# Nicolas-Zamorano/pytorch_fem_solver

Measured on AMD Instinct MI355X. Metric: Melements/s assembled (global K + f), higher is better.
Workload: dtype f64

## Files before the change

### include/tfem_assembly.h

```cpp
#ifndef TFEM_ASSEMBLY_H
#define TFEM_ASSEMBLY_H

#include <stdint.h>

#ifdef __cplusplus
extern "C" {
#endif

#define TFEM_ABI_VERSION 2

typedef enum tfem_status {
  TFEM_OK = 0,
  TFEM_ERR_INVALID_ARGUMENT = 1,
  TFEM_ERR_UNSUPPORTED = 2,
  TFEM_ERR_HIP = 3,
  TFEM_ERR_INDEX_RANGE = 4,
  TFEM_ERR_NO_DEVICE = 5
} tfem_status;

int tfem_abi_version(void);
const char *tfem_status_string(int status);
const char *tfem_last_error(void);
int tfem_device_count(void);
int tfem_quadrature_size(int quad_order);
// ... 125 lines not shown
  TFEM_SRC_SIN = 17, TFEM_SRC_COS = 18, TFEM_SRC_EXP = 19, TFEM_SRC_SQRT = 20,
  TFEM_SRC_LOG = 21, TFEM_SRC_TANH = 22,
  TFEM_SRC_OP_COUNT = 23
};
typedef struct tfem_source_program {
  int32_t n_ops;
  int32_t reserved;
  uint8_t ops[TFEM_SOURCE_MAX_OPS];
  double consts[TFEM_SOURCE_MAX_OPS];
} tfem_source_program;

int tfem_source_validate(const tfem_source_program *program);

int tfem_source_eval(const void *coords, int real_bytes, const void *conn, int idx_bytes,
                     int64_t n_elems, int64_t n_verts, int quad_order,
                     const tfem_source_program *program, void *fq, void *stream);

int tfem_p1_assemble_rings_source(const void *coords, int real_bytes, int64_t n_verts,
                                  int quad_order, double alpha, double beta,
                                  const void *plan_device, const int64_t *plan_layout_host,
                                  void *vals, int64_t nnz, const tfem_source_program *source,
                                  int64_t n_elems, void *fout, void *stream);

int tfem_p1_rings_coef(const void *coords, int real_bytes, int64_t n_verts, int quad_order,
                       double alpha, double beta, const tfem_source_program *kappa,
                       const tfem_source_program *c, const void *plan_device,
                       const int64_t *plan_layout_host, void *vals, void *stream);
int tfem_p1_apply_rings_coef(const void *coords, int real_bytes, int64_t n_verts, int quad_order,
                             double alpha, double beta, const tfem_source_program *kappa,
                             const tfem_source_program *c, const void *plan_device,
                             const int64_t *plan_layout_host, const void *u, void *y, void *stream);
int tfem_p1_apply_rings_coef_multi(const void *coords, int real_bytes, int64_t n_verts, int quad_order,
                                   double alpha, double beta, const tfem_source_program *kappa,
                                   const tfem_source_program *c, const void *plan_device,
                                   const int64_t *plan_layout_host, const void *u, void *y,
                                   int64_t n_vec, void *stream);

int tfem_p1_rings_field(const void *coords, int real_bytes, int64_t n_verts, int quad_order,
                        double alpha, double beta, const void *kappa, int kappa_nq, const void *c,
                        int c_nq, int64_t n_elems, const void *plan_device,
                        const int64_t *plan_layout_host, void *vals, void *stream);
int tfem_p1_apply_rings_field(const void *coords, int real_bytes, int64_t n_verts, int quad_order,
                              double alpha, double beta, const void *kappa, int kappa_nq,
                              const void *c, int c_nq, int64_t n_elems, const void *plan_device,
                              const int64_t *plan_layout_host, const void *u, void *y, void *stream);
int tfem_p1_field_adjoint(const void *coords, int real_bytes, const void *conn, int64_t n_elems,
// ... 70 lines not shown
```

### pytorch_fem_solver_amd/_native.py

```python

from __future__ import annotations

import ctypes
import os
from ctypes import c_char_p, c_double, c_int, c_int64, c_void_p

_HERE = os.path.dirname(os.path.abspath(__file__))
LIB_PATH = os.environ.get("TFEM_HIP_LIB") or os.path.join(_HERE, "csrc", "libtfem_hip.so")

_lib = None

ABI_VERSION = 2

SOURCE_MAX_OPS = 32
SOURCE_STACK = 4


class SourceProgram(ctypes.Structure):
    _fields_ = [
        ("n_ops", ctypes.c_int32),
        ("reserved", ctypes.c_int32),
        ("ops", ctypes.c_uint8 * SOURCE_MAX_OPS),
        ("consts", ctypes.c_double * SOURCE_MAX_OPS),
    ]
# ... 147 lines not shown
        c_int,
        [c_void_p, c_int, c_void_p, c_void_p, c_void_p, c_int64, c_int, c_void_p, c_void_p, c_void_p,
         c_void_p, c_void_p, c_int64, c_void_p],
    ),
    "tfem_edge_interpolate_p1_fracture": (
        c_int,
        [c_void_p, c_void_p, c_int, c_void_p, c_void_p, c_void_p, c_void_p, c_int64, c_int64, c_int64,
         c_int64, c_int, c_void_p, c_int64, c_void_p, c_void_p, c_void_p],
    ),
    "tfem_csr_gather_map": (c_int, [c_void_p, c_int64, c_int, c_int64, c_void_p, c_void_p]),
    "tfem_csr_gather": (c_int, [c_void_p, c_int, c_void_p, c_void_p, c_int64, c_void_p, c_void_p]),
    "tfem_interface_pack": (
        c_int,
        [c_void_p, c_void_p, c_int, c_void_p, c_void_p, c_int64, c_void_p, c_void_p, c_int64,
         c_void_p, c_int64, c_void_p],
    ),
    "tfem_interface_unpack": (
        c_int,
        [c_void_p, c_void_p, c_int, c_void_p, c_void_p, c_int64, c_void_p, c_void_p, c_int64,
         c_void_p, c_void_p],
    ),
    "tfem_interface_pack_dense": (c_int, [c_void_p, c_void_p, c_int, c_void_p, c_int64, c_void_p, c_void_p]),
    "tfem_source_validate": (c_int, [c_void_p]),
    "tfem_source_eval": (
        c_int,
        [c_void_p, c_int, c_void_p, c_int, c_int64, c_int64, c_int, c_void_p, c_void_p, c_void_p],
    ),
    "tfem_p1_assemble_rings_source": (
        c_int,
        [c_void_p, c_int, c_int64, c_int, c_double, c_double, c_void_p, c_void_p, c_void_p,
         c_int64, c_void_p, c_int64, c_void_p, c_void_p],
    ),
    "tfem_p1_rings_coef": (
        c_int,
        [c_void_p, c_int, c_int64, c_int, c_double, c_double, c_void_p, c_void_p, c_void_p, c_void_p,
         c_void_p, c_void_p],
    ),
    "tfem_p1_apply_rings_coef": (
        c_int,
        [c_void_p, c_int, c_int64, c_int, c_double, c_double, c_void_p, c_void_p, c_void_p, c_void_p,
         c_void_p, c_void_p, c_void_p],
    ),
    "tfem_p1_apply_rings_coef_multi": (
        c_int,
        [c_void_p, c_int, c_int64, c_int, c_double, c_double, c_void_p, c_void_p, c_void_p, c_void_p,
         c_void_p, c_void_p, c_int64, c_void_p],
# ... 79 lines not shown
```

### pytorch_fem_solver_amd/basis/engine.py

```python

from __future__ import annotations

import ctypes
import os
from ctypes import c_void_p

import numpy as np
import torch

from .. import _native
from ..sparse import CSRMatrix


class NoDeviceError(RuntimeError):
    pass


def _is_block(u):
    return u is not None and u.dim() == 2 and u.shape[1] > 1


def _compute_device(home: torch.device) -> torch.device:
    if home.type == "cuda":
        return home
    if torch.cuda.is_available():
        return torch.device("cuda", torch.cuda.current_device())
# ... 850 lines not shown
        out = torch.empty(out_len, dtype=self.dtype, device=self.device)
        with torch.cuda.device(self.device):
            _native.check(
                self.lib.tfem_tri_bilinear_csr(
                    _native.ptr(d["coords"]), self.real_bytes, _native.ptr(d["conn_geo"]), 4,
                    self.n_elems, self.coords_per_mesh, self.poly_order, self.quad_order,
                    float(alpha), float(beta), None if two_pass else _native.ptr(csr[2]),
                    _native.ptr(out), out_len,
                    _native.ptr(d["pinv"]), _native.ptr(d["fdet"]), self.n_fractures,
                    self.coords_per_mesh, self._stream(),
                )
            )
        return self._gather_local(out) if two_pass else out

    def _output(self, given, numel, what):
        if given is None:
            return torch.empty(numel, dtype=self.dtype, device=self.device)
        if (given.dtype != self.dtype or given.device != self.device or given.numel() != numel
                or not given.is_contiguous()):
            raise ValueError(f"out: {what} must be a contiguous {self.dtype} tensor of {numel} "
                             f"entries on {self.device}")
        return given.view(-1)

    def _assemble_rings(self, alpha, beta, fq=None, want_matrix=True, out=(None, None), source=None,
                        tiles=None):
        d = self._inputs()
        rings = self.ring_plan()
        nnz = int(self.csr_structure()[1].shape[0])
        vals = self._output(out[0], nnz, "CSR values") if want_matrix else None
        fout = None
        with_load = fq is not None or source is not None
        if fq is not None:
            fq = fq.to(self.device, self.dtype).reshape(self.n_elems, self.n_quad).contiguous()
        if with_load:
            fout = self._output(out[1], self.n_dofs, "load vector")
        with torch.cuda.device(self.device):
            if tiles is not None:
                _native.check(
                    self.lib.tfem_p1_assemble_rings_range(
                        _native.ptr(d["coords"]), self.real_bytes, self.n_dofs, self.quad_order,
                        float(alpha), float(beta), _native.ptr(rings["blob"]),
                        c_void_p(rings["layout"].ctypes.data), _native.ptr(vals), nnz,
                        _native.ptr(fq), ctypes.byref(source) if source is not None else None,
                        self.n_elems, _native.ptr(fout), int(tiles[0]), int(tiles[1]), self._stream(),
                    )
                )
            elif source is not None:
                _native.check(
                    self.lib.tfem_p1_assemble_rings_source(
                        _native.ptr(d["coords"]), self.real_bytes, self.n_dofs, self.quad_order,
                        float(alpha), float(beta), _native.ptr(rings["blob"]),
                        c_void_p(rings["layout"].ctypes.data), _native.ptr(vals), nnz,
                        ctypes.byref(source), self.n_elems, _native.ptr(fout), self._stream(),
                    )
                )
            else:
                _native.check(
                    self.lib.tfem_p1_assemble_rings(
# ... 362 lines not shown
        if (fq is None) == (source is None):
            raise ValueError("prepared_system: source values fq OR a source program")
        rings = self.ring_plan() if self._use_rings() else None
        if rings is None or (source is not None and not self._rings_take_source()) or (source is None and not rings["fq_ok"]):
            raise NotImplementedError("prepared launches need the ring plan of this basis")
        d = self._inputs()
        nnz = int(self.csr_structure()[1].shape[0])
        vals = self._output(out[0], nnz, "CSR values")
        fout = self._output(out[1], self.n_dofs, "load vector")
        first, count = self.tile_range(tiles) if tiles is not None else (0, -1)
        if fq is not None:
            fq = fq.to(self.device, self.dtype).reshape(self.n_elems, self.n_quad).contiguous()
        program = None
        if source is not None:
            program = _native.SourceProgram()
            ctypes.memmove(ctypes.byref(program), ctypes.byref(source), ctypes.sizeof(program))
        fixed = (_native.ptr(d["coords"]), self.real_bytes, self.n_dofs, self.quad_order, float(alpha), float(beta),
                 _native.ptr(rings["blob"]), c_void_p(rings["layout"].ctypes.data), _native.ptr(vals), nnz,
                 _native.ptr(fq), ctypes.byref(program) if program is not None else None, self.n_elems,
                 _native.ptr(fout), int(first), int(count))
        keep = (d, rings, vals, fout, fq, program)
        launch_fn, device, check = self.lib.tfem_p1_assemble_rings_range, self.device, _native.check
        current_stream = torch.cuda.current_stream

        def launch(stream=None):
            handle = (stream if stream is not None else current_stream(device)).cuda_stream
            status = launch_fn(*fixed, c_void_p(handle))
            if status:
                check(status)
            return keep[2], keep[3]

        return launch

    def supports_source(self):
        return self.n_fractures == 0 and self._host_coords.dim() == 2

    def _rings_take_source(self):
        if self.kernel == "tiles" or not self._use_rings():
            return False
        if os.environ.get("TFEM_DETERMINISTIC", "0") not in ("", "0"):
            return False
        rings = self.ring_plan()
        return bool(rings["elems_staged"] and rings["has_tverts"])

    def source_values(self, program):
        d = self._inputs()
        fq = torch.empty((self.n_elems, self.n_quad), dtype=self.dtype, device=self.device)
        with torch.cuda.device(self.device):
# ... 293 lines not shown
```

### pytorch_fem_solver_amd/csrc/tfem_rings.hip

```cpp
#include <cmath>

#include "tfem_rings_kernel.hpp"

namespace tfem {

template <typename T, bool MASS>
__global__ __launch_bounds__(kRingBlock) void k_p1_long_rows(const T *coords, const unsigned char *plan,
                                                             unsigned off_long, int n_long, T *vals, T stiff_w,
                                                             T mass_d, T mass_o) {
  RingLongSlot<T> s;
  ring_long_slot<T, MASS, false>(coords, plan, off_long, n_long, stiff_w, mass_o, nullptr, s);
  if (!s.slot) return;
  T *out = vals + s.rec[1];
  out[int((s.rec[19 + s.i / 8] >> (4 * (s.i % 8))) & 15u)] = s.entry;
  if (s.i == 0) out[s.dpos] = ring_diag<T, MASS>(s.sum, s.dsum, mass_d, mass_o);
}

struct RingLaunch {
  const void *coords;
  int quad_order;
  double alpha, beta;
  const unsigned char *plan;
  const int64_t *layout;
  int64_t n_verts, nnz;
// ... 22 lines not shown
static void *pick_ring_q(int nq) {
  switch (nq) {
    case 0: return reinterpret_cast<void *>(k_p1_rings<T, SLOTS, MASS, CHUNK, 0, false>);
    case 1: return reinterpret_cast<void *>(k_p1_rings<T, SLOTS, MASS, CHUNK, 1, false>);
    case 3: return reinterpret_cast<void *>(k_p1_rings<T, SLOTS, MASS, CHUNK, 3, false>);
    case 4: return reinterpret_cast<void *>(k_p1_rings<T, SLOTS, MASS, CHUNK, 4, false>);
    case 6: return reinterpret_cast<void *>(k_p1_rings<T, SLOTS, MASS, CHUNK, 6, false>);
    default: return nullptr;
  }
}

template <typename T, int SLOTS, bool CHUNK>
static void *pick_ring_mass(bool kmat, bool mass, int nq) {
  if (!kmat) return pick_ring_load_only<T, SLOTS, CHUNK>(nq);
  return mass ? pick_ring_q<T, SLOTS, true, CHUNK>(nq) : pick_ring_q<T, SLOTS, false, CHUNK>(nq);
}

template <typename T>
static void *pick_ring_kernel(int slots, bool mass, bool chunk, int nq, bool src, bool kmat, bool wide) {
  if (src) return pick_ring_src_kernel<T>(slots, mass, chunk, nq, kmat, wide);
  if (slots == 7)
    return chunk ? pick_ring_mass<T, 7, true>(kmat, mass, nq) : pick_ring_mass<T, 7, false>(kmat, mass, nq);
  return chunk ? pick_ring_mass<T, 15, true>(kmat, mass, nq) : pick_ring_mass<T, 15, false>(kmat, mass, nq);
}

template <typename T>
static int launch_rings(const RingLaunch &L) {
  TriTables tables;
  if (!build_tri_tables(L.quad_order, int(sizeof(T)), &tables))
    return fail(TFEM_ERR_UNSUPPORTED, "Integration order not implemented");
  const int64_t *z = L.layout;
  if (z[0] == 0) return TFEM_OK;
  const bool src = L.source != nullptr;
  const bool load = L.fq != nullptr || src;
  const bool kmat = L.vals != nullptr;
  if (src && L.fq) return fail(TFEM_ERR_INVALID_ARGUMENT, "source values AND a source program");
  if (!kmat && !load) return fail(TFEM_ERR_INVALID_ARGUMENT, "nothing to assemble");
  if (!L.coords || !L.plan || (load && !L.fout)) return fail(TFEM_ERR_INVALID_ARGUMENT, "NULL pointer");
  RingArgs<T> a;
  int st = ring_args_init<T>(tables, z, L.coords, L.plan, L.n_verts, L.alpha, L.beta, a);
  if (st != TFEM_OK) return st;
  const int64_t rb = int64_t(sizeof(T));
  const int64_t extents[3] = {kmat ? L.nnz * rb : 0, (load && !src) ? L.n_elems * tables.nq * rb : 0,
                              load ? L.n_verts * rb : 0};
  st = check_extents("ring kernel", extents, 3);
  if (st != TFEM_OK) return st;
// ... 30 lines not shown
    auto near = [tol](double x, double y) { return std::fabs(x - y) <= tol; };
    bool ok = tables.hw[1] == tables.hw[2] && tables.hw[1] == tables.hw[3];
    for (int i = 0; i < 3; ++i) {
      ok = ok && near(tables.lam[0][i], c0);
      for (int q = 1; q < 4; ++q) ok = ok && near(tables.lam[q][i], i == at[q] ? aa : b);
    }
    if (!ok) return fail(TFEM_ERR_UNSUPPORTED, "the 4-point rule is not the reference's order-3 rule");
    a.qsym[0] = T(c0);
    a.qsym[1] = T(b);
    a.qsym[2] = T(d);
    a.qsym[3] = T(c0) * T(tables.hw[0]);
    a.qsym[4] = T(b) * T(tables.hw[1]);
    a.qsym[5] = T(d) * T(tables.hw[1]);
  }
  if (src) {
    if (z[20] == 0 || z[21] == 0)
      return fail(TFEM_ERR_UNSUPPORTED, "the ring plan carries no element vertex table (source programs)");
    a.off_tverts = unsigned(z[20]);
    a.off_chain = unsigned(z[24]);
    a.off_hin = unsigned(z[26]);
    a.chain_len = int(z[25]);
    if (a.chain_len < 1 || z[24] == 0 || z[26] == 0)
      return fail(TFEM_ERR_INVALID_ARGUMENT, "the ring plan carries no chain order (layout of an older build?)");
    st = src_convert<T>(L.source, &a.src);
    if (st != TFEM_OK) return st;
  }
  const int64_t t_first = L.tile_first, t_count = L.tile_count < 0 ? z[0] - L.tile_first : L.tile_count;
  if (t_first < 0 || t_count < 0 || t_first + t_count > z[0])
    return fail(TFEM_ERR_INVALID_ARGUMENT, "tile range [%lld, +%lld) outside the plan's %lld tiles",
                (long long)t_first, (long long)t_count, (long long)z[0]);
  if (kmat && z[23] > 0 && (t_first != 0 || t_count != z[0]))
    return fail(TFEM_ERR_UNSUPPORTED, "a ring plan with long rows is launched over all of its tiles: the rows of "
                "the vertices with 8 .. 15 neighbours are written by one launch over all of them");
  if (t_count == 0) return TFEM_OK;
  a.n_tiles = int(t_count);
  a.n_runs = 0;
  if (src) {
    a.u_first = int(t_first);
    if (z[28] > 0 && (t_first != 0 || t_count != z[0]))
      return fail(TFEM_ERR_UNSUPPORTED, "tile ranges need a plan built with flagged vertices (its blocks break between the ranges)");
    if (z[28] > 0) {
      a.n_runs = int(z[28]);
      a.off_runs = unsigned(z[30]);
    }
  } else {
    a.off_desc += 80u * unsigned(t_first);
  }
  const bool mass = L.beta != 0.0;
  const int slots = int(z[6]);
  a.lds_elem = load ? int(z[17]) : 0;
  const size_t lds = size_t(4 * a.lds_vert) * sizeof(T) +
                     (kmat ? size_t(kRingWaves) * size_t(64 * (slots + 1) + 2) * sizeof(T) : 0) +
                     (src ? size_t(3 * (a.lds_vert + 2)) * sizeof(T)
                          : load ? size_t(3 * a.lds_elem + 4) * sizeof(T) : 0);
  const bool chunk = z[13] != 0;
  a.plain_stores = !load;
  if (const char *v = std::getenv("TFEM_RINGS_STORES")) a.plain_stores = std::strcmp(v, "plain") == 0;
  bool wide = src && src_depth(L.source) <= 2;
  if (const char *v = std::getenv("TFEM_SRC_WIDE")) wide = wide && std::atoi(v) != 0;
  void *kernel = pick_ring_kernel<T>(slots, mass, chunk, load ? tables.nq : 0, src, kmat, wide);
  if (!kernel) return fail(TFEM_ERR_UNSUPPORTED, "Integration order not implemented");
  int per_cu = 0;
  st = resident_per_cu(kernel, kRingBlock, lds, &per_cu);
  if (st != TFEM_OK) return st;
  const int deal = a.xcd_interleave > 0 ? a.xcd_interleave : 1;
  int per = int((t_count + 8 * deal - 1) / (8 * deal)) * deal;
  if (src) {
    const int64_t first_block = t_first / a.chain_len, last_block = (t_first + t_count - 1) / a.chain_len;
    per = int((last_block - first_block + 1 + 7) / 8);
    if (a.n_runs > 0) per = (a.n_runs + 7) / 8;
  }
  if (L.blocks_per_cu > 0 && L.blocks_per_cu < per_cu) per_cu = L.blocks_per_cu;
  int cus = device_cu_count();
  if (const char *v = std::getenv("TFEM_RINGS_RESERVE_CUS")) cus = std::max(8, cus - 8 * std::max(0, std::atoi(v)));
  const int blocks = std::min(per * 8, (cus * per_cu / 8) * 8);
  const dim3 grid{unsigned(blocks)}, block{unsigned(kRingBlock)};
  void *params[] = {&a};
  hipError_t e = hipLaunchKernel(kernel, grid, block, params, lds, L.stream);
  if (e != hipSuccess) return fail(TFEM_ERR_HIP, "ring kernel launch: %s", hipGetErrorString(e));
  if (kmat && z[23] > 0) {
    const dim3 lgrid{unsigned((16 * z[23] + kRingBlock - 1) / kRingBlock)};
    if (mass)
// ... 11 lines not shown
static int ring_entry(const void *coords, int real_bytes, int64_t n_verts, int quad_order, double alpha,
                      double beta, const void *plan_device, const int64_t *plan_layout_host, void *vals,
                      int64_t nnz, const void *fq, const tfem_source_program *source, int64_t n_elems,
                      void *fout, int64_t tile_first, int64_t tile_count, void *stream) {
  if (real_bytes != 4 && real_bytes != 8)
    return fail(TFEM_ERR_INVALID_ARGUMENT, "real_bytes must be 4 or 8");
  if (!plan_layout_host) return fail(TFEM_ERR_INVALID_ARGUMENT, "plan_layout_host is NULL");
  RingLaunch L{coords, quad_order, alpha, beta, static_cast<const unsigned char *>(plan_device),
               plan_layout_host, n_verts, nnz, vals, static_cast<hipStream_t>(stream)};
  L.fq = fq;
  L.source = source;
  L.n_elems = n_elems;
  L.fout = fout;
  L.tile_first = tile_first;
  L.tile_count = tile_count;
  if (const char *v = std::getenv("TFEM_RINGS_PER_CU")) L.blocks_per_cu = std::atoi(v);
  return real_bytes == 8 ? launch_rings<double>(L) : launch_rings<float>(L);
}

}

extern "C" {

int tfem_ring_capacity(int what) {
  using namespace tfem;
  switch (what) {
    case 0: return kRingBlock;
    case 1: return kRingVertCap;
    default: return 0;
  }
}

int tfem_p1_assemble_rings(const void *coords, int real_bytes, int64_t n_verts, int quad_order,
                           double alpha, double beta, const void *plan_device,
                           const int64_t *plan_layout_host, void *vals, int64_t nnz,
                           const void *fq, int64_t n_elems, void *fout, void *stream) {
  return tfem::ring_entry(coords, real_bytes, n_verts, quad_order, alpha, beta, plan_device, plan_layout_host, vals,
                          nnz, fq, nullptr, n_elems, fout, 0, -1, stream);
}

int tfem_p1_assemble_rings_source(const void *coords, int real_bytes, int64_t n_verts, int quad_order,
                                  double alpha, double beta, const void *plan_device,
                                  const int64_t *plan_layout_host, void *vals, int64_t nnz,
                                  const tfem_source_program *source, int64_t n_elems, void *fout,
                                  void *stream) {
  if (!source) return tfem::fail(TFEM_ERR_INVALID_ARGUMENT, "NULL pointer");
// ... 15 lines not shown
```

### pytorch_fem_solver_amd/csrc/tfem_rings_host.cpp

```cpp
#include <algorithm>
#include <cmath>
#include <cstdlib>
#include <cstring>
#include <memory>
#include <numeric>
#include <vector>
#include <chrono>
#include <cstdio>

#include "tfem_common.hpp"
#include "tfem_threads.hpp"

namespace tfem {

constexpr int kRingDescStride = 20;
constexpr int kRingLayoutLen = 32;
constexpr int kRingElemCap = 768;
constexpr int kRingElemRuns = 8;
constexpr int kRingHaloCapHost = 256;

struct RingPlan {
  int slots = 7, words = 4;
  std::vector<int32_t> desc;
  std::vector<uint32_t> rows;
// ... 1016 lines not shown
      {layout[9], p->rows.data(), int64_t(p->rows.size()) * 4},
      {layout[10], p->rowstart.data(), int64_t(p->rowstart.size()) * 4},
      {layout[11], p->vert_gid.data(), int64_t(p->vert_gid.size()) * 4},
      {layout[15], p->row_ecodes.data(), int64_t(p->row_ecodes.size()) * 4},
      {layout[16], p->tile_elems.data(), int64_t(p->tile_elems.size()) * 4},
      {layout[20], p->tile_tverts.data(), int64_t(p->tile_tverts.size()) * 4},
      {layout[22], p->long_rows.data(), int64_t(p->long_rows.size()) * 4},
      {layout[24], p->chain_order.data(), int64_t(p->chain_order.size()) * 4},
      {layout[26], p->hand_in.data(), int64_t(p->hand_in.size()) * 2},
      {layout[30], p->runs.data(), int64_t(p->runs.size()) * 4},
  };
  for (const Part &part : parts) {
    const int64_t padded = (part.bytes + 15) & ~int64_t(15);
    std::memset(out + part.off + part.bytes, 0, size_t(padded - part.bytes));
    if (part.bytes == 0) continue;
    parallel_for(part.bytes, [&](int64_t b, int64_t e, int) {
      std::memcpy(out + part.off + b, static_cast<const unsigned char *>(part.src) + b, size_t(e - b));
    }, 1 << 20);
  }
  std::memset(out + layout[12] - 64, 0, 64);
  return TFEM_OK;
}

void tfem_ring_plan_destroy(void *plan_handle) { delete static_cast<tfem::RingPlan *>(plan_handle); }

}
```

### pytorch_fem_solver_amd/csrc/tfem_rings_kernel.hpp

```cpp
#pragma once

#include <hip/hip_runtime.h>

#include <algorithm>
#include <cstdlib>
#include <cstring>
#include <type_traits>

#include "tfem_common.hpp"
#include "tfem_rowkit.hpp"
#include "tfem_source.hpp"

#pragma clang fp contract(fast)

namespace tfem {

constexpr int kRingBlock = 256;
constexpr int kRingWaves = kRingBlock / 64;
constexpr int kRingVertCap = 1024;

template <typename T>
struct RingArgs {
  const T *coords;
  const unsigned char *plan;
// ... 403 lines not shown
      v[q] = __builtin_bit_cast(double, ru32x2{x.x, x.y});
      v[q + 1] = __builtin_bit_cast(double, ru32x2{x.z, x.w});
    } else {
      v[q] = __builtin_bit_cast(float, __builtin_amdgcn_raw_buffer_load_b32(r, byte + unsigned(q) * 4u, 0, 0));
      v[q + 1] = __builtin_bit_cast(float, __builtin_amdgcn_raw_buffer_load_b32(r, byte + unsigned(q) * 4u + 4u, 0, 0));
    }
  }
  if (QL & 1) {
    const unsigned o = byte + unsigned(QL - 1) * unsigned(sizeof(T));
    if constexpr (sizeof(T) == 8) {
      const unsigned lo = __builtin_amdgcn_raw_buffer_load_b32(r, o, 0, 0);
      const unsigned hi = __builtin_amdgcn_raw_buffer_load_b32(r, o + 4u, 0, 0);
      v[QL > 0 ? QL - 1 : 0] = __builtin_bit_cast(double, ru32x2{lo, hi});
    } else {
      v[QL > 0 ? QL - 1 : 0] = __builtin_bit_cast(float, __builtin_amdgcn_raw_buffer_load_b32(r, o, 0, 0));
    }
  }
}

template <typename T, int SLOTS, bool MASS, bool CHUNK, int QL, bool, bool KMAT = true, int SRC = 0>
__global__ __launch_bounds__(kRingBlock, (SRC && SLOTS == 7 && QL <= 4) ? 4 : (SLOTS > 7 && QL == 0) ? 3 : 1) void k_p1_rings(const RingArgs<T> a) {
  constexpr bool LOAD = QL > 0;
  constexpr bool FQ = LOAD && !SRC;
  static_assert(KMAT || LOAD, "nothing to assemble");
  static_assert(LOAD || !SRC, "a source program needs a load vector");
  constexpr int kEW = (12 * SLOTS + 31) / 32;
  extern __shared__ __attribute__((aligned(16))) unsigned char ring_smem[];
  T *xy = reinterpret_cast<T *>(ring_smem);
  T *stage = xy + 4 * a.lds_vert;
  T *gtab = stage + (KMAT ? kRingWaves * ring_stage_entries<T, SLOTS>() : 0);
  const int tid = threadIdx.x;
  const int lane = tid & 63;
  const int wave = __builtin_amdgcn_readfirstlane(tid >> 6);
  T *my_stage = stage + wave * ring_stage_entries<T, SLOTS>();
  const int deal = a.xcd_interleave > 0 ? a.xcd_interleave : 1;
  const int per = (a.n_tiles + 8 * deal - 1) / (8 * deal) * deal;
  const int xcd = blockIdx.x & 7;
  const int j0 = blockIdx.x >> 3;
  const int stride = gridDim.x >> 3;
  const int clen = SRC ? a.chain_len : 1;
  const int u_end = a.u_first + a.n_tiles;
  const int block0 = SRC ? a.u_first / clen : 0;
  const bool balanced = SRC && a.n_runs > 0;
  int run = int(blockIdx.x) - int(gridDim.x), run_at = 0, run_end = 0;
  auto next_position = [&]() {
    while (run_at == run_end) {
// ... 243 lines not shown
            add_share((code >> (10 * i)) & 0x3FFu, acc, det * g);
          }
        }
      }
    }
  };

  auto load_tile = [&](const RingDesc &d, unsigned g_own, unsigned g_halo) {
    const int r = d.row0 + lane;
    const unsigned row = r < d.row1 ? unsigned(d.row_off + r) : kNone;
    ring_load_rec<SLOTS>(r_plan, a.off_rows + row * kRecBytes, rec_ld);
    if (!CHUNK)
      rowstart_ld = int(__builtin_amdgcn_raw_buffer_load_b32(r_plan, a.off_rowstart + row * 4u, 0, 0));
    if (FQ) {
      const unsigned eb = a.off_elems + row * unsigned(4 * kEW);
#pragma unroll
      for (int i = 0; i < kEW; i += 3) {
        const ru32x3 v = __builtin_amdgcn_raw_buffer_load_b96(r_plan, eb + unsigned(4 * i), 0, kStreamLoadNT);
        se_ld[FQ ? i : 0] = v.x;
        se_ld[FQ ? i + 1 : 0] = v.y;
        se_ld[FQ ? i + 2 : 0] = v.z;
      }
    }
    ring_load_xy<T>(r_coords, g_own, own_ld[0], own_ld[1]);
    ring_load_xy<T>(r_coords, g_halo, halo_ld[0], halo_ld[1]);
    if (SRC)
      hin_ld = __builtin_amdgcn_raw_buffer_load_b16(r_plan, a.off_hin + row * 2u, 0, 0);
  };
  auto park = [&](const RingDesc &d, T *dst) {
    const int r = d.row0 + lane;
    if (r < d.row1) {
      dst[2 * r] = own_ld[0];
      dst[2 * r + 1] = own_ld[1];
    }
    const int h = d.n_own + tid;
    if (h < d.n_vert) {
      dst[2 * h] = halo_ld[0];
      dst[2 * h + 1] = halo_ld[1];
    }
  };

  int t_c = tile_at(0);
  if (t_c < 0) return;
  int t_n = tile_at(1), t_nn = tile_at(2);
  RingDesc dc = ring_desc<CHUNK>(a.plan, a.off_desc, t_c, wave);
  RingDesc dn = ring_desc<CHUNK>(a.plan, a.off_desc, t_n >= 0 ? t_n : t_c, wave);
  RingDesc dnn = ring_desc<CHUNK>(a.plan, a.off_desc, t_nn >= 0 ? t_nn : t_c, wave);
  load_ids(dc, gid_own, gid_halo);
  load_eids(dc, eid);
  __builtin_amdgcn_s_waitcnt(0x0F70);
  load_tile(dc, gid_own, gid_halo);
  load_fq(dc, eid);
  load_tverts(dc, tev_ld, 0);
  if (t_n >= 0) {
    load_ids(dn, gid_own_ld, gid_halo_ld);
    load_eids(dn, eid_ld);
  }
  __builtin_amdgcn_s_waitcnt(0x0F70);
  park(dc, xy);
  park_g(dc, gtab);
  rec = rec_ld;
  hin = hin_ld;
  rowstart = rowstart_ld;
  gid_row = gid_own;
#pragma unroll
  for (int i = 0; i < (FQ ? kEW : 1); ++i) se[i] = se_ld[i];
#pragma unroll
  for (int j = 0; j < (FQ ? kRingElemPerLane : 1); ++j) eid[j] = eid_ld[j];
#pragma unroll
  for (int j = 0; j < (SRC ? kRingElemPerLane : 1); ++j) tev[j] = tev_ld[j];
  gid_own = gid_own_ld;
  gid_halo = gid_halo_ld;
  __syncthreads();

  int cur = 0;
  int a_cur = 0, a_prev = 2, a_next = 1;
  for (int k = 0;; ++k) {
    if (SRC) {
      switch ((k + int(blockIdx.x >> kRingPrioShift)) & 3) {
        case 0: __builtin_amdgcn_s_setprio(0); break;
        case 1: __builtin_amdgcn_s_setprio(1); break;
        case 2: __builtin_amdgcn_s_setprio(2); break;
        default: __builtin_amdgcn_s_setprio(3); break;
      }
    }
    auto phase_a = [&]() {
      if (t_n >= 0) {
        load_tile(dn, gid_own, gid_halo);
        load_fq(dn, eid);
        load_tverts(dn, tev_ld, k + 1);
        if (t_nn >= 0) {
          load_ids(dnn, gid_own_ld, gid_halo_ld);
          load_eids(dnn, eid_ld);
        }
      }
    };
    if (SRC) {
      compute_g(dc, tev, xy + cur * 2 * a.lds_vert, accs + a_cur * acc_stride, k);
    }
    phase_a();
    T off[SLOTS + 1], diag, sdets[SLOTS];
    constexpr int kBandSlots = (SLOTS > kRingBand && kRingBand > 0) ? kRingBand : (SLOTS == 7 && SRC ? 6 : SLOTS);
    const bool banded = kBandSlots < SLOTS && __builtin_amdgcn_ballot_w64(rec.k() > kBandSlots) == 0;
    bool regular = false;
    const int my_row = dc.row0 + lane;
    const uint32_t lv = unsigned(my_row < dc.row1 ? my_row : 0);
    if constexpr (SLOTS == 7 && SRC) {
      const bool mine = ((rec.w[2] >> 10) & 0x3FFFu) == 0x555u && rec.k() == 6;
      regular = __builtin_amdgcn_ballot_w64(!(mine || my_row >= dc.row1)) == 0;
    }
    if (regular) {
      if constexpr (SLOTS == 7) ring_row_regular<T, MASS>(a, rec, lv, xy + cur * 2 * a.lds_vert, off, diag);
    } else if (banded)
      ring_row<T, SLOTS, MASS, FQ, kBandSlots>(a, rec, lv, xy + cur * 2 * a.lds_vert, off, diag, sdets);
    else
      ring_row<T, SLOTS, MASS, FQ>(a, rec, lv, xy + cur * 2 * a.lds_vert, off, diag, sdets);
    int total = 0, pre = 0;
    if (KMAT) {
      if (regular) {
        if constexpr (SLOTS == 7) total = ring_stage_regular<T>(rec, off, diag, my_stage, pre, dc.row1 - dc.row0);
// ... 67 lines not shown
#pragma unroll
    for (int j = 0; j < (SRC ? kRingElemPerLane : 1); ++j) tev[j] = tev_ld[j];
    gid_own = gid_own_ld;
    gid_halo = gid_halo_ld;
    {
      const int t = a_prev;
      a_prev = a_cur;
      a_cur = a_next;
      a_next = t;
    }
    ring_lds_barrier();
    t_c = t_n;
    dc = dn;
    t_n = t_nn;
    dn = dnn;
    t_nn = tile_at(k + 3);
    if (t_nn >= 0) dnn = ring_desc<CHUNK>(a.plan, a.off_desc, t_nn, wave);
    cur ^= 1;
  }
}

template <typename T>
void *pick_ring_src_kernel(int slots, bool mass, bool chunk, int nq, bool kmat, bool wide);

template <typename T>
static int ring_args_init(const TriTables &tables, const int64_t *z, const void *coords, const unsigned char *plan,
                   int64_t n_verts, double alpha, double beta, RingArgs<T> &a) {
  if (z[0] < 0 || z[4] > kRingBlock || z[3] > kRingVertCap || z[4] > z[3] || z[14] > kRingHaloCap ||
      !((z[6] == 7 && z[7] == 4) || (z[6] == 15 && z[7] == 8)) || (z[5] > z[6] + 1 && z[23] == 0) || z[5] > 16)
    return fail(TFEM_ERR_INVALID_ARGUMENT, "ring plan exceeds the kernel's capacities");
  const int64_t extents[2] = {n_verts * 2 * int64_t(sizeof(T)), z[12]};
  const int st = check_extents("ring kernel", extents, 2);
  if (st != TFEM_OK) return st;
  std::memset(&a, 0, sizeof(a));
  a.coords = static_cast<const T *>(coords);
  a.plan = plan;
  a.coords_bytes = unsigned(extents[0]);
  a.plan_bytes = unsigned(extents[1]);
  a.off_desc = unsigned(z[8]);
  a.off_rows = unsigned(z[9]);
  a.off_rowstart = unsigned(z[10]);
  a.off_gid = unsigned(z[11]);
  a.n_tiles = int(z[0]);
  a.lds_vert = (int(z[3]) + 1) & ~1;
  T w = T(0), md = T(0), mo = T(0);
  for (int q = 0; q < tables.nq; ++q) {
// ... 12 lines not shown
```

### pytorch_fem_solver_amd/csrc/tfem_rings_src.hip

```cpp
#include "tfem_rings_kernel.hpp"

namespace tfem {

template <typename T, int SLOTS, bool CHUNK, int SRC>
static void *pick_src_load_only(int nq) {
  switch (nq) {
    case 1: return reinterpret_cast<void *>(k_p1_rings<T, SLOTS, false, CHUNK, 1, false, false, SRC>);
    case 3: return reinterpret_cast<void *>(k_p1_rings<T, SLOTS, false, CHUNK, 3, false, false, SRC>);
    case 4: return reinterpret_cast<void *>(k_p1_rings<T, SLOTS, false, CHUNK, 4, false, false, SRC>);
    case 6: return reinterpret_cast<void *>(k_p1_rings<T, SLOTS, false, CHUNK, 6, false, false, SRC>);
    default: return nullptr;
  }
}

template <typename T, int SLOTS, bool MASS, bool CHUNK, int SRC>
static void *pick_src_q(int nq) {
  switch (nq) {
    case 1: return reinterpret_cast<void *>(k_p1_rings<T, SLOTS, MASS, CHUNK, 1, false, true, SRC>);
    case 3: return reinterpret_cast<void *>(k_p1_rings<T, SLOTS, MASS, CHUNK, 3, false, true, SRC>);
    case 4: return reinterpret_cast<void *>(k_p1_rings<T, SLOTS, MASS, CHUNK, 4, false, true, SRC>);
    case 6: return reinterpret_cast<void *>(k_p1_rings<T, SLOTS, MASS, CHUNK, 6, false, true, SRC>);
    default: return nullptr;
  }
}

template <typename T, int SLOTS, bool CHUNK, int SRC>
static void *pick_src_mass(bool kmat, bool mass, int nq) {
  if (!kmat) return pick_src_load_only<T, SLOTS, CHUNK, SRC>(nq);
  return mass ? pick_src_q<T, SLOTS, true, CHUNK, SRC>(nq) : pick_src_q<T, SLOTS, false, CHUNK, SRC>(nq);
}

template <typename T, int SRC>
static void *pick_src_slots(int slots, bool mass, bool chunk, int nq, bool kmat) {
  if (slots == 7)
    return chunk ? pick_src_mass<T, 7, true, SRC>(kmat, mass, nq) : pick_src_mass<T, 7, false, SRC>(kmat, mass, nq);
  return chunk ? pick_src_mass<T, 15, true, SRC>(kmat, mass, nq) : pick_src_mass<T, 15, false, SRC>(kmat, mass, nq);
}

template <typename T>
void *pick_ring_src_kernel(int slots, bool mass, bool chunk, int nq, bool kmat, bool wide) {
  if (wide && nq <= 4) return pick_src_slots<T, 2>(slots, mass, chunk, nq, kmat);
  return pick_src_slots<T, 1>(slots, mass, chunk, nq, kmat);
}

template void *pick_ring_src_kernel<double>(int, bool, bool, int, bool, bool);
template void *pick_ring_src_kernel<float>(int, bool, bool, int, bool, bool);

}
```

### pytorch_fem_solver_amd/csrc/tfem_source.hip

```cpp
#include <hip/hip_runtime.h>

#include <cstring>

#include "tfem_common.hpp"
#include "tfem_source.hpp"

namespace tfem {

int src_validate(const tfem_source_program *in) {
  if (!in) return fail(TFEM_ERR_INVALID_ARGUMENT, "source program is NULL");
  if (in->n_ops < 1 || in->n_ops > kSrcMaxOps)
    return fail(TFEM_ERR_INVALID_ARGUMENT, "source program: %d operations (1..%d)", in->n_ops, kSrcMaxOps);
  int depth = 0;
  for (int i = 0; i < in->n_ops; ++i) {
    const int op = in->ops[i];
    int pops = 0, pushes = 0;
    switch (op) {
      case TFEM_SRC_PUSH_X: case TFEM_SRC_PUSH_Y: case TFEM_SRC_PUSH_C: pushes = 1; break;
      case TFEM_SRC_ADD: case TFEM_SRC_SUB: case TFEM_SRC_SUB_R: case TFEM_SRC_MUL:
      case TFEM_SRC_DIV: case TFEM_SRC_DIV_R: pops = 2; pushes = 1; break;
      case TFEM_SRC_ADD_C: case TFEM_SRC_MUL_C: case TFEM_SRC_RSUB_C: case TFEM_SRC_RDIV_C:
      case TFEM_SRC_NEG: case TFEM_SRC_ABS: case TFEM_SRC_SIN: case TFEM_SRC_COS:
      case TFEM_SRC_EXP: case TFEM_SRC_SQRT: case TFEM_SRC_LOG: case TFEM_SRC_TANH:
        pops = 1; pushes = 1; break;
// ... 22 lines not shown
      ++depth;
    else if (op >= TFEM_SRC_ADD && op <= TFEM_SRC_DIV_R)
      --depth;
    peak = depth > peak ? depth : peak;
  }
  return peak;
}

template <typename T>
int src_convert(const tfem_source_program *in, SrcProgram<T> *out) {
  const int st = src_validate(in);
  if (st != TFEM_OK) return st;
  std::memset(out, 0, sizeof(*out));
  out->n_ops = in->n_ops;
  for (int i = 0; i < in->n_ops; ++i) {
    out->opw[i >> 2] |= uint32_t(in->ops[i]) << (8 * (i & 3));
    out->c[i] = T(in->consts[i]);
  }
  return TFEM_OK;
}
template int src_convert<double>(const tfem_source_program *, SrcProgram<double> *);
template int src_convert<float>(const tfem_source_program *, SrcProgram<float> *);

namespace {

constexpr int kSrcBlock = 256;

template <typename T, typename I>
struct SrcEvalArgs {
  const T *coords;
  const I *conn;
  T *fq;
  int64_t n_elems;
  T lam[3][kMaxQuad];
  SrcProgram<T> src;
};

template <typename T, typename I, int Q>
__global__ __launch_bounds__(kSrcBlock) void k_source_eval(const SrcEvalArgs<T, I> a) {
  const int64_t e = int64_t(blockIdx.x) * kSrcBlock + threadIdx.x;
  const int64_t ec = e < a.n_elems ? e : a.n_elems - 1;
  const I *c = a.conn + 3 * ec;
  const int64_t v0 = c[0], v1 = c[1], v2 = c[2];
  const T x0 = a.coords[2 * v0], y0 = a.coords[2 * v0 + 1];
  const T x1 = a.coords[2 * v1], y1 = a.coords[2 * v1 + 1];
  const T x2 = a.coords[2 * v2], y2 = a.coords[2 * v2 + 1];
// ... 29 lines not shown
  const int st = src_convert<T>(program, &a.src);
  if (st != TFEM_OK) return st;
  if (n_elems == 0) return TFEM_OK;
  const dim3 grid(unsigned((n_elems + kSrcBlock - 1) / kSrcBlock)), block(kSrcBlock);
  switch (tables.nq) {
    case 1: hipLaunchKernelGGL((k_source_eval<T, I, 1>), grid, block, 0, stream, a); break;
    case 3: hipLaunchKernelGGL((k_source_eval<T, I, 3>), grid, block, 0, stream, a); break;
    case 4: hipLaunchKernelGGL((k_source_eval<T, I, 4>), grid, block, 0, stream, a); break;
    case 6: hipLaunchKernelGGL((k_source_eval<T, I, 6>), grid, block, 0, stream, a); break;
    default: return fail(TFEM_ERR_UNSUPPORTED, "Integration order not implemented");
  }
  const hipError_t e = hipGetLastError();
  if (e != hipSuccess) return fail(TFEM_ERR_HIP, "source evaluation launch: %s", hipGetErrorString(e));
  return TFEM_OK;
}

}
}

extern "C" {

int tfem_source_validate(const tfem_source_program *program) { return tfem::src_validate(program); }

int tfem_source_eval(const void *coords, int real_bytes, const void *conn, int idx_bytes,
                     int64_t n_elems, int64_t n_verts, int quad_order,
                     const tfem_source_program *program, void *fq, void *stream) {
  using namespace tfem;
  if ((real_bytes != 4 && real_bytes != 8) || (idx_bytes != 4 && idx_bytes != 8))
    return fail(TFEM_ERR_INVALID_ARGUMENT, "real_bytes / idx_bytes must be 4 or 8");
  if (n_elems < 0 || n_verts < 0 || (n_elems > 0 && (!coords || !conn || !fq)))
    return fail(TFEM_ERR_INVALID_ARGUMENT, "bad arguments");
  hipStream_t s = static_cast<hipStream_t>(stream);
  if (real_bytes == 8)
    return idx_bytes == 4 ? run_source_eval<double, int32_t>(coords, conn, n_elems, quad_order, program, fq, s)
                          : run_source_eval<double, int64_t>(coords, conn, n_elems, quad_order, program, fq, s);
  return idx_bytes == 4 ? run_source_eval<float, int32_t>(coords, conn, n_elems, quad_order, program, fq, s)
                        : run_source_eval<float, int64_t>(coords, conn, n_elems, quad_order, program, fq, s);
}

}
```

### pytorch_fem_solver_amd/csrc/tfem_source.hpp

```cpp
#pragma once

#include <hip/hip_runtime.h>

#include <cstddef>
#include <cstdint>

#include "tfem_assembly.h"

namespace tfem {

constexpr int kSrcMaxOps = TFEM_SOURCE_MAX_OPS;
constexpr int kSrcStack = TFEM_SOURCE_STACK;

template <typename T>
struct SrcProgram {
  int n_ops;
  int pad;
  uint32_t opw[kSrcMaxOps / 4];
  T c[kSrcMaxOps];
};

template <typename T>
int src_convert(const tfem_source_program *in, SrcProgram<T> *out);
int src_validate(const tfem_source_program *in);
int src_depth(const tfem_source_program *in);

#if defined(__HIPCC__)

template <typename T>
__device__ __forceinline__ T src_fma(T a, T b, T c) {
  if constexpr (sizeof(T) == 8) return __builtin_fma(a, b, c);
  else return __builtin_fmaf(a, b, c);
}

__device__ __forceinline__ double src_sin_poly(double r) {
  const double r2 = r * r;
  double p = 2.73144475909634011e-15;
  p = __builtin_fma(p, r2, -7.64397029616579265e-13);
  p = __builtin_fma(p, r2, 1.60589773124442683e-10);
  p = __builtin_fma(p, r2, -2.50521076169958777e-08);
  p = __builtin_fma(p, r2, 2.75573192191632300e-06);
  p = __builtin_fma(p, r2, -1.98412698412549741e-04);
  p = __builtin_fma(p, r2, 8.33333333333331587e-03);
  p = __builtin_fma(p, r2, -1.66666666666666657e-01);
  return __builtin_fma(r * r2, p, r);
}

__device__ __forceinline__ double src_sin_poly_scaled(double r, double c) {
// ... 288 lines not shown
                                             const T (&lam_arg)[3][kMaxQuad], size_t lam_offset,
                                             T (&out)[NE * QL]) {
  constexpr int N = NE * QL;
  T s0[N], s1[N];
#pragma unroll
  for (int i = 0; i < N; ++i) asm volatile("" : "=v"(s0[i]), "=v"(s1[i]));
  const int n = prog.n_ops;
  int depth = 0;
#define TFEM_SRC_SET(expr)             \
  _Pragma("unroll") for (int i = 0; i < N; ++i) { \
    const T t = s0[i];                 \
    const T l = s1[i];                 \
    (void)t;                           \
    (void)l;                           \
    s0[i] = (expr);                    \
  }
#pragma unroll 1
  for (int pc = 0; pc < n; ++pc) {
    const uint32_t op = uint32_t(__builtin_amdgcn_readlane(int(prog.op), pc));
    const T c = src_lane_const<T>(prog, pc);
    if (op <= TFEM_SRC_PUSH_C) {
      if (depth > 0) {
#pragma unroll
        for (int i = 0; i < N; ++i) s1[i] = s0[i];
      }
      depth = __builtin_amdgcn_readfirstlane(depth + 1);
    } else if (op <= TFEM_SRC_DIV_R) {
      depth = __builtin_amdgcn_readfirstlane(depth - 1);
    }
    switch (op) {
#define TFEM_SRC_PUSH_COORD(comp)                                                                    \
  {                                                                                                  \
    T lam[3][QL];                                                                                    \
    if constexpr (kSrcTableLoads<T>) {                                                               \
      const src_const_tab<T> ltab = src_kernarg_table<T>(lam_offset);                                \
      _Pragma("unroll") for (int k = 0; k < 3; ++k)                                                  \
        _Pragma("unroll") for (int q = 0; q < QL; ++q) lam[k][q] = ltab[k * kMaxQuad + q];           \
    } else {                                                                                         \
      _Pragma("unroll") for (int k = 0; k < 3; ++k)                                                  \
        _Pragma("unroll") for (int q = 0; q < QL; ++q) lam[k][q] = lam_arg[k][q];                    \
    }                                                                                                \
    T vert[NE][3];                                                                                   \
    _Pragma("unroll") for (int e = 0; e < NE; ++e)                                                   \
      _Pragma("unroll") for (int k = 0; k < 3; ++k) vert[e][k] = vert_at[e][k][comp];                \
    _Pragma("unroll") for (int e = 0; e < NE; ++e)                                                   \
      _Pragma("unroll") for (int q = 0; q < QL; ++q)  \
        s0[e * QL + q] =                                                                             \
// ... 10 lines not shown
      case TFEM_SRC_DIV: TFEM_SRC_SET(l / t) break;
      case TFEM_SRC_DIV_R: TFEM_SRC_SET(t / l) break;
      case TFEM_SRC_ADD_C: TFEM_SRC_SET(t + c) break;
      case TFEM_SRC_MUL_C: TFEM_SRC_SET(t * c) break;
      case TFEM_SRC_RSUB_C: TFEM_SRC_SET(c - t) break;
      case TFEM_SRC_RDIV_C: TFEM_SRC_SET(c / t) break;
      case TFEM_SRC_NEG: TFEM_SRC_SET(-t) break;
      case TFEM_SRC_ABS:
        if constexpr (sizeof(T) == 8) { TFEM_SRC_SET(__builtin_fabs(t)) } else { TFEM_SRC_SET(__builtin_fabsf(t)) }
        break;
      case TFEM_SRC_POW_I: {
        const int e = int(c);
#pragma unroll
        for (int i = 0; i < N; ++i) {
          const T t = s0[i];
          T r = t * t;
          for (int k = 2; k < e; ++k) r = r * t;
          s0[i] = r;
        }
        break;
      }
      case TFEM_SRC_SIN: src_sin_scaled<T, N>(s0, c); break;
      case TFEM_SRC_COS: src_cos_scaled<T, N>(s0, c); break;
      case TFEM_SRC_EXP:
        if constexpr (sizeof(T) == 8) { TFEM_SRC_WIDE_APPLY(s0, exp) } else { TFEM_SRC_WIDE_APPLY(s0, expf) }
        TFEM_SRC_SET(c * t)
        break;
      case TFEM_SRC_SQRT:
        if constexpr (sizeof(T) == 8) { TFEM_SRC_SET(c * sqrt(t)) } else { TFEM_SRC_SET(c * sqrtf(t)) }
        break;
      case TFEM_SRC_LOG:
        if constexpr (sizeof(T) == 8) { TFEM_SRC_WIDE_APPLY(s0, log) } else { TFEM_SRC_WIDE_APPLY(s0, logf) }
        TFEM_SRC_SET(c * t)
        break;
      case TFEM_SRC_TANH:
        if constexpr (sizeof(T) == 8) { TFEM_SRC_WIDE_APPLY(s0, tanh) } else { TFEM_SRC_WIDE_APPLY(s0, tanhf) }
        TFEM_SRC_SET(c * t)
        break;
      default: break;
    }
  }
#undef TFEM_SRC_SET
#pragma unroll
  for (int i = 0; i < N; ++i) out[i] = s0[i];
}

// ... 4 lines not shown
```

Baseline: 66650.

## Prove trig argument bounds from coordinate range and stage source coords via LDS DMA

```diff
diff --git a/include/tfem_assembly.h b/include/tfem_assembly.h
--- a/include/tfem_assembly.h
+++ b/include/tfem_assembly.h
@@ -171,6 +171,15 @@
                                   void *vals, int64_t nnz, const tfem_source_program *source,
                                   int64_t n_elems, void *fout, void *stream);
 
+int tfem_ring_plan_vouch_coords(int64_t *plan_layout_host, const void *coords, double max_abs_coord);
+
+int tfem_p1_rings_source_ops(const void *coords, int real_bytes, int quad_order,
+                             const int64_t *plan_layout_host, const tfem_source_program *source,
+                             uint8_t *ops_out);
+
+int tfem_source_trig_proof(const tfem_source_program *program, double max_abs_coord,
+                           uint8_t *fast_out);
+
 int tfem_p1_rings_coef(const void *coords, int real_bytes, int64_t n_verts, int quad_order,
                        double alpha, double beta, const tfem_source_program *kappa,
                        const tfem_source_program *c, const void *plan_device,
diff --git a/pytorch_fem_solver_amd/_native.py b/pytorch_fem_solver_amd/_native.py
--- a/pytorch_fem_solver_amd/_native.py
+++ b/pytorch_fem_solver_amd/_native.py
@@ -193,6 +193,9 @@
     ),
     "tfem_interface_pack_dense": (c_int, [c_void_p, c_void_p, c_int, c_void_p, c_int64, c_void_p, c_void_p]),
     "tfem_source_validate": (c_int, [c_void_p]),
+    "tfem_source_trig_proof": (c_int, [c_void_p, c_double, c_void_p]),
+    "tfem_ring_plan_vouch_coords": (c_int, [c_void_p, c_void_p, c_double]),
+    "tfem_p1_rings_source_ops": (c_int, [c_void_p, c_int, c_int, c_void_p, c_void_p, c_void_p]),
     "tfem_source_eval": (
         c_int,
         [c_void_p, c_int, c_void_p, c_int, c_int64, c_int64, c_int, c_void_p, c_void_p, c_void_p],
diff --git a/pytorch_fem_solver_amd/basis/engine.py b/pytorch_fem_solver_amd/basis/engine.py
--- a/pytorch_fem_solver_amd/basis/engine.py
+++ b/pytorch_fem_solver_amd/basis/engine.py
@@ -2,6 +2,7 @@
 from __future__ import annotations
 
 import ctypes
+import math
 import os
 from ctypes import c_void_p
 
@@ -898,6 +899,26 @@
                              f"entries on {self.device}")
         return given.view(-1)
 
+    def _vouch_ring_coords(self, rings, coords):
+        state = rings.get("coords_version")
+        version = coords._version
+        if state == version:
+            return
+        layout = c_void_p(rings["layout"].ctypes.data)
+        if state is None:
+            if torch.cuda.is_current_stream_capturing():
+                return
+            bound = 0.0
+            if coords.numel():
+                lo, hi = torch.aminmax(coords)
+                bound = max(abs(float(lo)), abs(float(hi)))
+            _native.check(self.lib.tfem_ring_plan_vouch_coords(layout, _native.ptr(coords),
+                                                               bound if math.isfinite(bound) else -1.0))
+            rings["coords_version"] = version
+        elif state != "withdrawn":
+            _native.check(self.lib.tfem_ring_plan_vouch_coords(layout, None, -1.0))
+            rings["coords_version"] = "withdrawn"
+
     def _assemble_rings(self, alpha, beta, fq=None, want_matrix=True, out=(None, None), source=None,
                         tiles=None):
         d = self._inputs()
@@ -910,6 +931,8 @@
             fq = fq.to(self.device, self.dtype).reshape(self.n_elems, self.n_quad).contiguous()
         if with_load:
             fout = self._output(out[1], self.n_dofs, "load vector")
+        if source is not None:
+            self._vouch_ring_coords(rings, d["coords"])
         with torch.cuda.device(self.device):
             if tiles is not None:
                 _native.check(
@@ -1318,8 +1341,13 @@
         keep = (d, rings, vals, fout, fq, program)
         launch_fn, device, check = self.lib.tfem_p1_assemble_rings_range, self.device, _native.check
         current_stream = torch.cuda.current_stream
+        coords, vouch = d["coords"], self._vouch_ring_coords
+        if program is not None:
+            vouch(rings, coords)
 
         def launch(stream=None):
+            if program is not None and coords._version != rings.get("coords_version"):
+                vouch(rings, coords)
             handle = (stream if stream is not None else current_stream(device)).cuda_stream
             status = launch_fn(*fixed, c_void_p(handle))
             if status:
diff --git a/pytorch_fem_solver_amd/csrc/tfem_rings.hip b/pytorch_fem_solver_amd/csrc/tfem_rings.hip
--- a/pytorch_fem_solver_amd/csrc/tfem_rings.hip
+++ b/pytorch_fem_solver_amd/csrc/tfem_rings.hip
@@ -68,6 +68,34 @@
   if (slots == 7)
     return chunk ? pick_ring_mass<T, 7, true>(kmat, mass, nq) : pick_ring_mass<T, 7, false>(kmat, mass, nq);
   return chunk ? pick_ring_mass<T, 15, true>(kmat, mass, nq) : pick_ring_mass<T, 15, false>(kmat, mass, nq);
+}
+
+static bool ring_src_wide(const tfem_source_program *source) {
+  bool wide = src_depth(source) <= 2;
+  if (const char *v = std::getenv("TFEM_SRC_WIDE")) wide = wide && std::atoi(v) != 0;
+  return wide;
+}
+
+template <typename T>
+static int ring_src_convert(const int64_t *z, const void *coords, int nq, const tfem_source_program *source,
+                            SrcProgram<T> *out) {
+  double coord_bound = -1.0;
+  if (z[29] != 0 && uintptr_t(z[29]) == reinterpret_cast<uintptr_t>(coords))
+    std::memcpy(&coord_bound, &z[31], sizeof(coord_bound));
+  if (sizeof(T) == 8 && coord_bound >= 0.0 && ring_src_runs_wide(nq, ring_src_wide(source)))
+    return src_convert_proven<T>(source, coord_bound, out);
+  return src_convert<T>(source, out);
+}
+
+template <typename T>
+static int ring_src_ops(const int64_t *z, const void *coords, int nq, const tfem_source_program *source,
+                        uint8_t *ops_out) {
+  SrcProgram<T> device;
+  const int st = ring_src_convert<T>(z, coords, nq, source, &device);
+  if (st != TFEM_OK) return st;
+  std::memset(ops_out, 0, kSrcMaxOps);
+  for (int i = 0; i < device.n_ops; ++i) ops_out[i] = uint8_t((device.opw[i >> 2] >> (8 * (i & 3))) & 0xFFu);
+  return TFEM_OK;
 }
 
 template <typename T>
@@ -144,7 +172,7 @@
     a.chain_len = int(z[25]);
     if (a.chain_len < 1 || z[24] == 0 || z[26] == 0)
       return fail(TFEM_ERR_INVALID_ARGUMENT, "the ring plan carries no chain order (layout of an older build?)");
-    st = src_convert<T>(L.source, &a.src);
+    st = ring_src_convert<T>(z, L.coords, tables.nq, L.source, &a.src);
     if (st != TFEM_OK) return st;
   }
   const int64_t t_first = L.tile_first, t_count = L.tile_count < 0 ? z[0] - L.tile_first : L.tile_count;
@@ -178,8 +206,7 @@
   const bool chunk = z[13] != 0;
   a.plain_stores = !load;
   if (const char *v = std::getenv("TFEM_RINGS_STORES")) a.plain_stores = std::strcmp(v, "plain") == 0;
-  bool wide = src && src_depth(L.source) <= 2;
-  if (const char *v = std::getenv("TFEM_SRC_WIDE")) wide = wide && std::atoi(v) != 0;
+  const bool wide = src && ring_src_wide(L.source);
   void *kernel = pick_ring_kernel<T>(slots, mass, chunk, load ? tables.nq : 0, src, kmat, wide);
   if (!kernel) return fail(TFEM_ERR_UNSUPPORTED, "Integration order not implemented");
   int per_cu = 0;
@@ -237,6 +264,18 @@
 
 extern "C" {
 
+int tfem_p1_rings_source_ops(const void *coords, int real_bytes, int quad_order, const int64_t *plan_layout_host,
+                             const tfem_source_program *source, uint8_t *ops_out) {
+  using namespace tfem;
+  if (real_bytes != 4 && real_bytes != 8) return fail(TFEM_ERR_INVALID_ARGUMENT, "real_bytes must be 4 or 8");
+  if (!plan_layout_host || !source || !ops_out) return fail(TFEM_ERR_INVALID_ARGUMENT, "NULL pointer");
+  TriTables tables;
+  if (!build_tri_tables(quad_order, real_bytes, &tables))
+    return fail(TFEM_ERR_UNSUPPORTED, "Integration order not implemented");
+  return real_bytes == 8 ? ring_src_ops<double>(plan_layout_host, coords, tables.nq, source, ops_out)
+                         : ring_src_ops<float>(plan_layout_host, coords, tables.nq, source, ops_out);
+}
+
 int tfem_ring_capacity(int what) {
   using namespace tfem;
   switch (what) {
diff --git a/pytorch_fem_solver_amd/csrc/tfem_rings_host.cpp b/pytorch_fem_solver_amd/csrc/tfem_rings_host.cpp
--- a/pytorch_fem_solver_amd/csrc/tfem_rings_host.cpp
+++ b/pytorch_fem_solver_amd/csrc/tfem_rings_host.cpp
@@ -1062,6 +1062,18 @@
   return TFEM_OK;
 }
 
+int tfem_ring_plan_vouch_coords(int64_t *plan_layout_host, const void *coords, double max_abs_coord) {
+  if (!plan_layout_host) return tfem::fail(TFEM_ERR_INVALID_ARGUMENT, "plan_layout_host is NULL");
+  int64_t bits = 0, array = 0;
+  if (coords && max_abs_coord >= 0.0 && std::isfinite(max_abs_coord)) {
+    std::memcpy(&bits, &max_abs_coord, sizeof(bits));
+    array = int64_t(reinterpret_cast<uintptr_t>(coords));
+  }
+  plan_layout_host[29] = array;
+  plan_layout_host[31] = bits;
+  return TFEM_OK;
+}
+
 void tfem_ring_plan_destroy(void *plan_handle) { delete static_cast<tfem::RingPlan *>(plan_handle); }
 
 }
diff --git a/pytorch_fem_solver_amd/csrc/tfem_rings_kernel.hpp b/pytorch_fem_solver_amd/csrc/tfem_rings_kernel.hpp
--- a/pytorch_fem_solver_amd/csrc/tfem_rings_kernel.hpp
+++ b/pytorch_fem_solver_amd/csrc/tfem_rings_kernel.hpp
@@ -449,6 +449,7 @@
 __global__ __launch_bounds__(kRingBlock, (SRC && SLOTS == 7 && QL <= 4) ? 4 : (SLOTS > 7 && QL == 0) ? 3 : 1) void k_p1_rings(const RingArgs<T> a) {
   constexpr bool LOAD = QL > 0;
   constexpr bool FQ = LOAD && !SRC;
+  constexpr bool kCoordsToLds = SRC == 2 && sizeof(T) == 8;
   static_assert(KMAT || LOAD, "nothing to assemble");
   static_assert(LOAD || !SRC, "a source program needs a load vector");
   constexpr int kEW = (12 * SLOTS + 31) / 32;
@@ -738,12 +739,15 @@
         se_ld[FQ ? i + 2 : 0] = v.z;
       }
     }
-    ring_load_xy<T>(r_coords, g_own, own_ld[0], own_ld[1]);
-    ring_load_xy<T>(r_coords, g_halo, halo_ld[0], halo_ld[1]);
+    if constexpr (!kCoordsToLds) {
+      ring_load_xy<T>(r_coords, g_own, own_ld[0], own_ld[1]);
+      ring_load_xy<T>(r_coords, g_halo, halo_ld[0], halo_ld[1]);
+    }
     if (SRC)
       hin_ld = __builtin_amdgcn_raw_buffer_load_b16(r_plan, a.off_hin + row * 2u, 0, 0);
   };
   auto park = [&](const RingDesc &d, T *dst) {
+    if constexpr (kCoordsToLds) return;
     const int r = d.row0 + lane;
     if (r < d.row1) {
       dst[2 * r] = own_ld[0];
@@ -753,6 +757,16 @@
     if (h < d.n_vert) {
       dst[2 * h] = halo_ld[0];
       dst[2 * h + 1] = halo_ld[1];
+    }
+  };
+  auto load_xy_lds = [&](const RingDesc &d, unsigned g_own, unsigned g_halo, T *dst) {
+    if constexpr (kCoordsToLds) {
+      typedef __attribute__((address_space(3))) void *lds_ptr;
+      if (d.row0 + lane < d.row1)
+        __builtin_amdgcn_raw_ptr_buffer_load_lds(r_coords, (lds_ptr)(dst + 2 * d.row0), 16, g_own * 16u, 0, 0, 0);
+      if (d.n_own + tid < d.n_vert)
+        __builtin_amdgcn_raw_ptr_buffer_load_lds(r_coords, (lds_ptr)(dst + 2 * (d.n_own + 64 * wave)), 16,
+                                                 g_halo * 16u, 0, 0, 0);
     }
   };
 
@@ -766,6 +780,7 @@
   load_eids(dc, eid);
   __builtin_amdgcn_s_waitcnt(0x0F70);
   load_tile(dc, gid_own, gid_halo);
+  load_xy_lds(dc, gid_own, gid_halo, xy);
   load_fq(dc, eid);
   load_tverts(dc, tev_ld, 0);
   if (t_n >= 0) {
@@ -812,6 +827,7 @@
       }
     };
     if (SRC) {
+      if (t_n >= 0) load_xy_lds(dn, gid_own, gid_halo, xy + (cur ^ 1) * 2 * a.lds_vert);
       compute_g(dc, tev, xy + cur * 2 * a.lds_vert, accs + a_cur * acc_stride, k);
     }
     phase_a();
@@ -925,6 +941,7 @@
 
 template <typename T>
 void *pick_ring_src_kernel(int slots, bool mass, bool chunk, int nq, bool kmat, bool wide);
+inline bool ring_src_runs_wide(int nq, bool wide) { return wide && nq <= 4; }
 
 template <typename T>
 static int ring_args_init(const TriTables &tables, const int64_t *z, const void *coords, const unsigned char *plan,
diff --git a/pytorch_fem_solver_amd/csrc/tfem_rings_src.hip b/pytorch_fem_solver_amd/csrc/tfem_rings_src.hip
--- a/pytorch_fem_solver_amd/csrc/tfem_rings_src.hip
+++ b/pytorch_fem_solver_amd/csrc/tfem_rings_src.hip
@@ -39,7 +39,7 @@
 
 template <typename T>
 void *pick_ring_src_kernel(int slots, bool mass, bool chunk, int nq, bool kmat, bool wide) {
-  if (wide && nq <= 4) return pick_src_slots<T, 2>(slots, mass, chunk, nq, kmat);
+  if (ring_src_runs_wide(nq, wide)) return pick_src_slots<T, 2>(slots, mass, chunk, nq, kmat);
   return pick_src_slots<T, 1>(slots, mass, chunk, nq, kmat);
 }
 
diff --git a/pytorch_fem_solver_amd/csrc/tfem_source.hip b/pytorch_fem_solver_amd/csrc/tfem_source.hip
--- a/pytorch_fem_solver_amd/csrc/tfem_source.hip
+++ b/pytorch_fem_solver_amd/csrc/tfem_source.hip
@@ -1,5 +1,6 @@
 #include <hip/hip_runtime.h>
 
+#include <cmath>
 #include <cstring>
 
 #include "tfem_common.hpp"
@@ -68,6 +69,40 @@
 template int src_convert<double>(const tfem_source_program *, SrcProgram<double> *);
 template int src_convert<float>(const tfem_source_program *, SrcProgram<float> *);
 
+int src_trig_proof(const tfem_source_program *in, double coord_bound, uint8_t (&fast)[kSrcMaxOps]) {
+  std::memset(fast, 0, sizeof(fast));
+  if (!in || in->n_ops < 1 || in->n_ops > kSrcMaxOps) return 0;
+  if (!(coord_bound >= 0.0) || !std::isfinite(coord_bound)) return 0;
+  int proven = 0;
+  for (int i = 1; i < in->n_ops; ++i) {
+    const int op = in->ops[i], before = in->ops[i - 1];
+    if (op != TFEM_SRC_SIN && op != TFEM_SRC_COS) continue;
+    if (before != TFEM_SRC_PUSH_X && before != TFEM_SRC_PUSH_Y) continue;
+    const double arg = std::fabs(in->consts[i - 1]) * coord_bound * (1.0 + 1e-9);
+    if (arg < kSrcTrigFastMax / 2) {
+      fast[i] = 1;
+      ++proven;
+    }
+  }
+  return proven;
+}
+
+template <typename T>
+int src_convert_proven(const tfem_source_program *in, double coord_bound, SrcProgram<T> *out) {
+  const int st = src_convert<T>(in, out);
+  if (st != TFEM_OK || sizeof(T) != 8) return st;
+  uint8_t fast[kSrcMaxOps];
+  if (src_trig_proof(in, coord_bound, fast) == 0) return st;
+  for (int i = 0; i < in->n_ops; ++i)
+    if (fast[i]) {
+      const uint32_t op = in->ops[i] == TFEM_SRC_SIN ? kSrcSinProven : kSrcCosProven;
+      out->opw[i >> 2] = (out->opw[i >> 2] & ~(0xFFu << (8 * (i & 3)))) | (op << (8 * (i & 3)));
+    }
+  return st;
+}
+template int src_convert_proven<double>(const tfem_source_program *, double, SrcProgram<double> *);
+template int src_convert_proven<float>(const tfem_source_program *, double, SrcProgram<float> *);
+
 namespace {
 
 constexpr int kSrcBlock = 256;
@@ -143,6 +178,15 @@
 
 int tfem_source_validate(const tfem_source_program *program) { return tfem::src_validate(program); }
 
+int tfem_source_trig_proof(const tfem_source_program *program, double max_abs_coord, uint8_t *fast_out) {
+  if (!fast_out) return 0;
+  uint8_t fast[tfem::kSrcMaxOps] = {};
+  int proven = 0;
+  if (program && tfem::src_validate(program) == TFEM_OK) proven = tfem::src_trig_proof(program, max_abs_coord, fast);
+  std::memcpy(fast_out, fast, sizeof(fast));
+  return proven;
+}
+
 int tfem_source_eval(const void *coords, int real_bytes, const void *conn, int idx_bytes,
                      int64_t n_elems, int64_t n_verts, int quad_order,
                      const tfem_source_program *program, void *fq, void *stream) {
diff --git a/pytorch_fem_solver_amd/csrc/tfem_source.hpp b/pytorch_fem_solver_amd/csrc/tfem_source.hpp
--- a/pytorch_fem_solver_amd/csrc/tfem_source.hpp
+++ b/pytorch_fem_solver_amd/csrc/tfem_source.hpp
@@ -24,6 +24,11 @@
 int src_convert(const tfem_source_program *in, SrcProgram<T> *out);
 int src_validate(const tfem_source_program *in);
 int src_depth(const tfem_source_program *in);
+
+constexpr int kSrcSinProven = TFEM_SRC_OP_COUNT, kSrcCosProven = TFEM_SRC_OP_COUNT + 1;
+int src_trig_proof(const tfem_source_program *in, double coord_bound, uint8_t (&fast)[kSrcMaxOps]);
+template <typename T>
+int src_convert_proven(const tfem_source_program *in, double coord_bound, SrcProgram<T> *out);
 
 #if defined(__HIPCC__)
 
@@ -358,7 +363,10 @@
     if (op <= TFEM_SRC_PUSH_C) {
       if (depth > 0) {
 #pragma unroll
-        for (int i = 0; i < N; ++i) s1[i] = s0[i];
+        for (int i = 0; i < N; ++i) {
+          s1[i] = s0[i];
+          asm volatile("" : "+v"(s1[i]));
+        }
       }
       depth = __builtin_amdgcn_readfirstlane(depth + 1);
     } else if (op <= TFEM_SRC_DIV_R) {
@@ -415,6 +423,12 @@
       }
       case TFEM_SRC_SIN: src_sin_scaled<T, N>(s0, c); break;
       case TFEM_SRC_COS: src_cos_scaled<T, N>(s0, c); break;
+      case kSrcSinProven:
+        if constexpr (sizeof(T) == 8) { TFEM_SRC_SET(src_sin_fast_scaled(t, c)) } else { src_sin_scaled<T, N>(s0, c); }
+        break;
+      case kSrcCosProven:
+        if constexpr (sizeof(T) == 8) { TFEM_SRC_SET(src_cos_fast_scaled(t, c)) } else { src_cos_scaled<T, N>(s0, c); }
+        break;
       case TFEM_SRC_EXP:
         if constexpr (sizeof(T) == 8) { TFEM_SRC_WIDE_APPLY(s0, exp) } else { TFEM_SRC_WIDE_APPLY(s0, expf) }
         TFEM_SRC_SET(c * t)
```

New measurement: 68830, median of 6. 1.03x the previous value.
